# adrianstanea/UnitSpeech

Hardware: AMD Instinct MI355X
Metric: mel-frames/sec @ 50 diffusion steps, 80x1024 (higher is better)
Workload: dtype f32; 1 GPU; B=1 utterance(s)/GPU, 80x1024 mel, 50 diffusion steps, text+spk CFG (3 score evals/step), full-size decoder (119.1M params, synthetic weights), built-in Philox noise; batch_per_gpu=1, frames=1024, diffusion_steps=50, parallelism=utterance-sharded x1

## Files before the change

unitspeech_amd/csrc/conv_igemm.hip:

```cpp
#include <type_traits>
#include "kernels.h"
#include "pack_f16.h"

namespace us {

typedef float f32x16 __attribute__((ext_vector_type(16)));
typedef float f32x4 __attribute__((ext_vector_type(4)));
typedef _Float16 half8 __attribute__((ext_vector_type(8)));

constexpr int TN = 128;

__device__ __forceinline__ void blds16(__amdgpu_buffer_rsrc_t rsrc, unsigned voff_bytes, unsigned soff_bytes, float* lds_dst_wave_uniform) {
  __builtin_amdgcn_raw_ptr_buffer_load_lds(rsrc, (__attribute__((address_space(3))) void*)lds_dst_wave_uniform, 16, (int)voff_bytes,
                                           (int)soff_bytes, 0, 0);
}

template <int BK, int WM, bool WINO, bool F16 = false, int NWM = 2, int NSTG = 2, bool ASPLIT = false, int NB = 2>
__global__ __launch_bounds__(NWM * 128, 2) void conv_igemm_kernel(ConvArgs a) {
  constexpr int TN = 64 * NB;
  constexpr int NW = 2 * NWM;
  constexpr int TM = NWM * WM;
  constexpr int MB = WM / 32;
  constexpr int CPR = BK / 4;
  constexpr int RPI = 64 / CPR;
  constexpr int IA = TM / RPI / NW;
  constexpr int IB = TN / RPI / NW;
  static_assert(NSTG == 2 || NSTG == 3, "two or three operand buffers");
  constexpr int SWZ_DIV = 64 / BK;
  constexpr int BUF = (TM + TN) * BK;
  extern __shared__ __attribute__((aligned(16))) float smem[];

  const int tid = threadIdx.x, lane = tid & 63;
// ... 431 lines not shown
#pragma unroll
    for (int mb = 0; mb < MB; ++mb)
#pragma unroll
      for (int r = 0; r < 16; ++r) {
        const int m = m0 + wm * WM + mb * 32 + (r & 3) + 8 * (r >> 2) + 4 * hh;
        if (m < Ms) {
#pragma unroll
          for (int nb = 0; nb < NB; ++nb) {
            const int n = n0 + wn * (32 * NB) + nb * 32 + l32;
            if (n < a.Cout) slab[(long long)m * a.Cout + n] = acc[mb][nb][r];
          }
        }
      }
    return;
  }
  __syncthreads();
  if constexpr (!WINO && MB == 1 && NB == 2) {
    if (a.attn_part_ctx && n0 >= a.attn_q_cols) {
      const int h = ((n0 - a.attn_q_cols) / TN) * 2 + wn;
      float* xm = smem;
      float* xs = smem + 128;
      float* xc = smem + 256;
      const int mrow0 = m0 + wm * WM + 4 * hh;
      float kmax = -INFINITY;
#pragma unroll
      for (int mb = 0; mb < MB; ++mb)
#pragma unroll
        for (int r = 0; r < 16; ++r) {
          const bool ok = mrow0 + mb * 32 + (r & 3) + 8 * (r >> 2) < Ms;
          kmax = fmaxf(kmax, ok ? acc[mb][0][r] : -INFINITY);
// ... 28 lines not shown
        float* pc = a.attn_part_ctx + (blk * kHeads + h) * (kDimHead * kDimHead);
#pragma unroll
        for (int r = 0; r < 16; ++r) {
          const int d = (r & 3) + 8 * (r >> 2) + 4 * hh;
          pc[d * kDimHead + l32] = ctx[r] + xc[wn * 1024 + d * 32 + l32];
        }
        if (hh == 0) {
          a.attn_part_m[blk * kHidden + h * kDimHead + l32] = mcol;
          a.attn_part_s[blk * kHidden + h * kDimHead + l32] = ssum + xs[wn * 32 + l32];
        }
      }
      return;
    }
  }
  float* tr = smem + wave * (32 * 36);
  const bool need_xy = !dense || om_b != nullptr;
  const int trow = lane >> 3, tc4 = (lane & 7) * 4;
  const bool edge = WINO && (((a.Hout | a.Wout) & 1) != 0);
  bool out_over = false;
  float bias_col[NB];
  f32x4 bias_quad[NB];
#pragma unroll
  for (int nb = 0; nb < NB; ++nb) {
    const int ncol = n0 + wn * (32 * NB) + nb * 32;
    bias_col[nb] = (a.bias && ncol + l32 < a.Cout) ? a.bias[ncol + l32] : 0.f;
    bias_quad[nb] = f32x4{0.f, 0.f, 0.f, 0.f};
    if (a.bias && ncol + tc4 < a.Cout) bias_quad[nb] = *reinterpret_cast<const f32x4*>(a.bias + ncol + tc4);
  }
#pragma unroll
  for (int yi = 0; yi < NY; ++yi) {
  const f32x16 (&A)[MB][NB] = WINO ? Y[yi] : acc;
  const int oy0 = WINO ? (yi >> 1) : a_oy0, ox0 = WINO ? (yi & 1) : a_ox0;
#pragma unroll
  for (int mb = 0; mb < MB; ++mb) {
    const int m_base = m0 + wm * WM + mb * 32;
    int yb = 0, xb = 0;
    if (need_xy) { yb = m_base / a.Ws; xb = m_base - yb * a.Ws; }
#pragma unroll
    for (int nb = 0; nb < NB; ++nb) {
      const int ncol = n0 + wn * (32 * NB) + nb * 32;
      {
        const int n = ncol + l32;
// ... 17 lines not shown
#pragma unroll
      for (int k = 0; k < 4; ++k) {
        const int dr = trow + 8 * k;
        const int m = m_base + dr;
        f32x4 v = *reinterpret_cast<const f32x4*>(tr + dr * 36 + tc4);
        if (m < Ms && n < a.Cout) {
          int yy = yb, xx = xb + dr;
          if (need_xy) while (xx >= a.Ws) { xx -= a.Ws; ++yy; }
          const int ox = ox0 + xx * a.ostep;
          const int oy = oy0 + yy * a.ostep;
          if (edge && (oy >= a.Hout || ox >= a.Wout)) continue;
          const long long pix = dense ? (long long)m : (long long)oy * a.Wout + ox;
          v = v + b4;
          if (a.out2) *reinterpret_cast<f32x4*>(a.out2 + ((long long)b * a.Hout * a.Wout + pix) * a.out2_ld + n) = v;
          v = v * alpha;
          if (add_b) v += *reinterpret_cast<const f32x4*>(add_b + pix * a.add_ld + n);
          if (om_b) v *= om_b[ox * a.omask_step];
          if (a.out_split) {
            typedef _Float16 half4o __attribute__((ext_vector_type(4)));
            half4o hi, lo;
#pragma unroll
            for (int q = 0; q < 4; ++q) {
              us_half h_, l_;
              split_f16x3(v[q], h_, l_, out_over);
              hi[q] = h_;
              lo[q] = l_;
            }
            _Float16* oh = reinterpret_cast<_Float16*>(out_b + pix * a.out_ld) + 2 * (n & ~7) + (n & 7);
            *reinterpret_cast<half4o*>(oh) = hi;
            *reinterpret_cast<half4o*>(oh + 8) = lo;
          } else {
// ... 24 lines not shown
      }
    }
  }
#ifdef US_LIFE
  US_LIFE_AT(4);
  US_LIFE_AT(3);
  if (a.stamp_out && lane == 0) {
    unsigned long long* o = a.stamp_out + ((blockIdx.x + gridDim.x * blockIdx.z) * NW + wave) * 4;
    o[0] = life_t[0]; o[1] = life_t[1]; o[2] = life_t[2]; o[3] = life_t[3];
  }
#endif
}

__global__ __launch_bounds__(256) void splitk_finish_kernel(ConvArgs a) {
  __shared__ double s_g[kGroups][2];
  const int b = blockIdx.y;
  const int Ms = a.Hs * a.Ws;
  const int C4 = a.Cout >> 2;
  const long long total = (long long)Ms * C4;
  if (threadIdx.x < kGroups * 2) s_g[threadIdx.x >> 1][threadIdx.x & 1] = 0.0;
  __syncthreads();
  float t1[4] = {0.f, 0.f, 0.f, 0.f}, t2[4] = {0.f, 0.f, 0.f, 0.f};
  int tn = -1;
  const bool dense = (a.ostep == 1 && a.oy0 == 0 && a.ox0 == 0 && a.Hs == a.Hout && a.Ws == a.Wout);
  const float alpha = a.alpha ? *a.alpha : 1.f;
  float* out_b = a.out + (long long)b * a.Hout * a.Wout * a.out_ld;
  const float* add_b = a.add ? a.add + (long long)b * a.Hout * a.Wout * a.add_ld : nullptr;
  const float* om_b = a.omask ? a.omask + (long long)(b % a.omask_bmod) * a.omask_ld : nullptr;
  const long long slice = (long long)a.B * Ms * a.Cout;
  const int cg = a.Cout / kGroups;
  for (long long i = blockIdx.x * 256LL + threadIdx.x; i < total; i += (long long)gridDim.x * 256) {
    const int n = (int)(i % C4) * 4;
    const int m = (int)(i / C4);
    const float* p = a.splitk_ws + ((long long)b * Ms + m) * a.Cout + n;
    f32x4 v = *reinterpret_cast<const f32x4*>(p);
    int k = 1;
    for (; k + 8 <= a.ksplit; k += 8) {
      f32x4 u[8];
#pragma unroll
      for (int j = 0; j < 8; ++j) u[j] = *reinterpret_cast<const f32x4*>(p + (k + j) * slice);
#pragma unroll
      for (int j = 0; j < 8; ++j) v += u[j];
    }
// ... 5 lines not shown
        for (int k = 0; k < 4; ++k) {
          atomicAdd(&s_g[(tn + k) / cg][0], (double)t1[k]);
          atomicAdd(&s_g[(tn + k) / cg][1], (double)t2[k]);
          t1[k] = t2[k] = 0.f;
        }
      }
      tn = n;
#pragma unroll
      for (int k = 0; k < 4; ++k) { t1[k] += v[k]; t2[k] += v[k] * v[k]; }
    }
    const int yy = m / a.Ws, xx = m - yy * a.Ws;
    const int ox = a.ox0 + xx * a.ostep;
    const long long pix = dense ? (long long)m : (long long)(a.oy0 + yy * a.ostep) * a.Wout + ox;
    if (a.out2) *reinterpret_cast<f32x4*>(a.out2 + ((long long)b * a.Hout * a.Wout + pix) * a.out2_ld + n) = v;
    v *= alpha;
    if (add_b) v += *reinterpret_cast<const f32x4*>(add_b + pix * a.add_ld + n);
    if (om_b) v *= om_b[ox * a.omask_step];
    *reinterpret_cast<f32x4*>(out_b + pix * a.out_ld + n) = v;
  }
  if (a.stats) {
    if (tn >= 0) {
#pragma unroll
      for (int k = 0; k < 4; ++k) {
        atomicAdd(&s_g[(tn + k) / cg][0], (double)t1[k]);
        atomicAdd(&s_g[(tn + k) / cg][1], (double)t2[k]);
      }
    }
    __syncthreads();
    if (threadIdx.x < kGroups * 2)
      stat_add(a.stats, b, threadIdx.x >> 1, threadIdx.x & 1, blockIdx.x, s_g[threadIdx.x >> 1][threadIdx.x & 1]);
  }
// ... 10 lines not shown
hipError_t conv_igemm_init() {
  hipError_t e;
  if ((e = set_attr<32, 64, false>()) != hipSuccess) return e;
  if ((e = set_attr<32, 32, false>()) != hipSuccess) return e;
  if ((e = set_attr<16, 64, false>()) != hipSuccess) return e;
  if ((e = set_attr<16, 32, false>()) != hipSuccess) return e;
  if ((e = set_attr<32, 32, true>()) != hipSuccess) return e;
  if ((e = set_attr<32, 64, false, true>()) != hipSuccess) return e;
  if ((e = set_attr<32, 64, false, true, 4, 3>()) != hipSuccess) return e;
  if ((e = hipFuncSetAttribute(reinterpret_cast<const void*>(&conv_igemm_kernel<32, 64, false, true, 4, 3, false, 1>),
                               hipFuncAttributeMaxDynamicSharedMemorySize, (int)lds_bytes(32, 256, 3, 64))) != hipSuccess) return e;
  if ((e = set_attr<32, 64, false, true, 4, 3, true>()) != hipSuccess) return e;
  if ((e = set_attr<32, 64, false, true, 2, 2, true>()) != hipSuccess) return e;
  if ((e = set_attr<32, 32, false, true, 2, 2, true>()) != hipSuccess) return e;
  if ((e = set_attr<32, 32, false, true>()) != hipSuccess) return e;
  if ((e = set_attr<32, 32, true, true, 2, 3>()) != hipSuccess) return e;
  return set_attr<16, 32, true>();
}

hipError_t launch_conv_igemm(const ConvArgs& a_in, hipStream_t s) {
  ConvArgs a = a_in;
  a.range_flag = current_range_flag();
  if (a.B <= 0 || a.Hs <= 0 || a.Ws <= 0) return hipSuccess;
  if (!a.in || !a.wt || !a.out) return hipErrorInvalidValue;
  if ((a.bk != 16 && a.bk != 32) || a.Cin % a.bk != 0 || a.ntaps < 1 || a.ntaps > kMaxTaps) return hipErrorInvalidValue;
  if (a.in_ld % 4 != 0) return hipErrorInvalidValue;
  if (a.Cout % 4 != 0 || a.out_ld % 4 != 0 || (a.add && a.add_ld % 4 != 0)) return hipErrorInvalidValue;
  if ((long long)a.Hin * a.Win * a.in_ld * 4 >= (1LL << 31) || (long long)kMaxTaps * a.Cout * a.Cin * 4 >= (1LL << 31))
    return hipErrorInvalidValue;
  if (a.stats) {
    int cg = a.Cout / kGroups;
    if (a.Cout % kGroups != 0 || (cg & (cg - 1)) != 0) return hipErrorInvalidValue;
  }
  if (a.out2 && (a.out2_ld % 4 != 0 || a.wino_out || a.out_split || a.attn_part_ctx)) return hipErrorInvalidValue;
  const int Ms = a.Hs * a.Ws;
  int tn = TN;
  int nt = (a.Cout + TN - 1) / TN;
  int tm = a.tm;
  if (a.f16) {
    if (a.bk != 32) return hipErrorInvalidValue;
    if (a.f16 == 1 && !a.direct_presplit && a.ntaps == 1 && a.istride == 1 && !a.bias && !a.add) a.splitk_ws = nullptr;
    if (tm == 0) {
      if (a.f16 == 1 && (a.ntaps > 1 || a.direct_presplit)) {
        tm = (a.ntaps == 1 && a.nphase <= 1) || (long long)a.Hs * a.Ws < 512 ? 64 : 128;
      } else if (a.f16 == 1) {
        const long long per256 = (long long)((a.Hs * a.Ws + 255) / 256) * nt * a.B;
        const long long per128 = (long long)((a.Hs * a.Ws + 127) / 128) * nt * a.B;
        const long long cost256 = ((per256 + 255) / 256) * 256, cost128 = ((per128 + 255) / 256) * 128;
        constexpr int kTmModelMargin = 15;
// ... 35 lines not shown
  const int mt = (Ms + tm - 1) / tm;
  const long long tiles = (long long)mt * nt * a.B;
  const int S_all = a.ntaps * (a.Cin / a.bk);
  a.ksplit = 1;
  const long long tiles_item = a.splitk_by_batch ? tiles : (long long)mt * nt;
  if (a.splitk_ws && tiles_item < 128 && S_all >= 8 && a.Cout % 4 == 0 && a.out_ld % 4 == 0 && (!a.add || a.add_ld % 4 == 0)) {
    long long k = (256 + tiles_item - 1) / tiles_item;
    if (k > S_all / 4) k = S_all / 4;
    if (k > 512 / tiles_item) k = 512 / tiles_item;
    if (k > 32) k = 32;
    if (k >= 2 && k * (long long)a.B * Ms * a.Cout <= a.splitk_ws_floats) a.ksplit = (int)k;
  }
  a.nt = nt;
  dim3 grid(mt * a.ksplit * nt, 1, a.B * (a.nphase > 1 ? a.nphase : 1));
  const size_t lds = lds_bytes(a.bk, tm);
  if (a.f16 == 2) {
    if (tm == 256) hipLaunchKernelGGL((conv_igemm_kernel<32, 64, false, true, 4, 3, true>), grid, dim3(512), lds_bytes(32, 256, 3), s, a);
    else if (tm == 128) hipLaunchKernelGGL((conv_igemm_kernel<32, 64, false, true, 2, 2, true>), grid, dim3(256), lds, s, a);
    else hipLaunchKernelGGL((conv_igemm_kernel<32, 32, false, true, 2, 2, true>), grid, dim3(256), lds, s, a);
  } else if (a.f16) {
    if (a.wino_out) hipLaunchKernelGGL((conv_igemm_kernel<32, 32, true, true, 2, 3>), grid, dim3(256), lds_bytes(32, 64, 3), s, a);
    else if (tm == 256 && tn == 64) hipLaunchKernelGGL((conv_igemm_kernel<32, 64, false, true, 4, 3, false, 1>), grid, dim3(512), lds_bytes(32, 256, 3, 64), s, a);
    else if (tm == 256) hipLaunchKernelGGL((conv_igemm_kernel<32, 64, false, true, 4, 3>), grid, dim3(512), lds_bytes(32, 256, 3), s, a);
    else if (tm == 128) hipLaunchKernelGGL((conv_igemm_kernel<32, 64, false, true>), grid, dim3(256), lds, s, a);
    else hipLaunchKernelGGL((conv_igemm_kernel<32, 32, false, true>), grid, dim3(256), lds, s, a);
  } else if (a.wino_out) {
    if (a.bk == 32)
      hipLaunchKernelGGL((conv_igemm_kernel<32, 32, true>), grid, dim3(256), lds, s, a);
    else
      hipLaunchKernelGGL((conv_igemm_kernel<16, 32, true>), grid, dim3(256), lds, s, a);
  } else if (a.bk == 32 && tm == 128)
// ... 66 lines not shown
```

unitspeech_amd/csrc/decoder.hip:

```cpp
#include <hip/hip_runtime.h>

#include <cmath>
#include <cstdarg>
#include <cstdio>
#include <cstring>
#include <algorithm>
#include <map>
#include <memory>
#include <string>
#include <vector>

#include "../../include/unitspeech_hip.h"
#include "kernels.h"
#include "pack_f16.h"

using namespace us;

namespace {

thread_local std::string g_last_error;

struct DevBuf {
  float* p = nullptr;
  size_t n = 0;
// ... 73 lines not shown
  std::vector<int> C;
  struct Down { ResnetW r1, r2; AttnW a; bool has_ds; ResampleW ds; };
  struct Up { ResnetW r1, r2; AttnW a; ResampleW us; };
  std::vector<Down> downs;
  ResnetW mid1, mid2;
  AttnW mid_attn;
  std::vector<Up> ups;
  ConvW final_conv3;
  Slot *final_g, *final_b, *final_w1, *final_b1;
  Slot *text_uncon, *spk_uncon, *mlp0_w, *mlp0_b, *mlp2_w, *mlp2_b;
  int n_resnets = 0;
  int wino_min_level = 1;
  int wino4_level_form[8] = {0, 0, 0, 0, 0, 0, 0, 0};
  int wino_fuse = -1;
  bool wino_fuse_gn = true;
  int f16_tm = 0;
  int wgrad_side_streams = 1;
  std::vector<hipStream_t> wgrad_streams;
  std::vector<hipEvent_t> wgrad_events;
  bool training = false;
  float* zeros = nullptr;
  unsigned* range_flag = nullptr;
  unsigned* range_host = nullptr;
  bool exact = false;
  float* grad_scale = nullptr;
  CopyEnt* grad_tab_dev = nullptr;
  static constexpr size_t kLinJobs = 64;
  LinJob *lin_tab_dev = nullptr, *lin_tab_bwd_dev = nullptr;
  std::vector<CopyEnt> pending_copies;
  std::vector<PackJob> pending_packs;
// ... 442 lines not shown
  if (w.w->wino.p && e.b->wino_v) return in_split ? hipErrorInvalidValue : conv3x3_wino(e, w, in, in_ld, level, out, out_ld, stats);
  const int H = e.h->cfg.n_feats >> level, W = e.T >> level;
  ConvArgs a = base_args(e, w, in, in_ld, H, W, out, out_ld, H, W);
  if (in_split) {
    if (a.f16 != 2) return hipErrorInvalidValue;
    a.f16 = 1;
    a.direct_presplit = 1;
  }
  a.ntaps = 9;
  for (int ky = 0; ky < 3; ++ky)
    for (int kx = 0; kx < 3; ++kx) a.set_tap(ky * 3 + kx, ky - 1, kx - 1, ky * 3 + kx);
  a.stats = stats;
  return run_conv(e, a);
}

hipError_t conv1x1(EvalCtx& e, const ConvW& w, const float* in, int in_ld, int level, bool mask_out, float* out, int out_ld,
                   const float* add, int add_ld, const float* alpha, const float* wt_override, long long wt_bstride,
                   const float* bias_override, bool in_split = false, bool out_split = false, float* out2 = nullptr, int out2_ld = 0) {
  const int H = e.h->cfg.n_feats >> level, W = e.T >> level;
  ConvArgs a = base_args(e, w, in, in_ld, H, W, out, out_ld, H, W);
  a.out2 = out2; a.out2_ld = out2_ld;
  if (in_split) {
    if (a.f16 != 2) return hipErrorInvalidValue;
    a.f16 = 1;
    a.direct_presplit = 1;
  }
  a.out_split = out_split ? 1 : 0;
  a.ntaps = 1;
  a.set_tap(0, 0, 0, 0);
  if (mask_out) set_omask(e, a, level);
  a.add = add; a.add_ld = add_ld; a.alpha = alpha;
  if (wt_override) { a.wt = wt_override; a.wt_bstride = wt_bstride; a.bias = bias_override; }
  return run_conv(e, a);
}

hipError_t conv_down(EvalCtx& e, const ConvW& w, const float* in, int in_ld, int level, float* out, int out_ld, bool in_split = false) {
  const int H = e.h->cfg.n_feats >> level, W = e.T >> level;
  ConvArgs a = base_args(e, w, in, in_ld, H, W, out, out_ld, H / 2, W / 2);
  if (in_split) {
    if (a.f16 != 2) return hipErrorInvalidValue;
    a.f16 = 1;
    a.direct_presplit = 1;
  }
  a.ntaps = 9;
  a.istride = 2;
  for (int ky = 0; ky < 3; ++ky)
// ... 78 lines not shown
    WinoGnArgs g{};
    g.stats = st1; g.gamma = r.g1->buf.p; g.beta = r.b1->buf.p; g.temb = tproj;
    g.mask = e.mask; g.mask_ld = e.T; g.mask_step = 1 << l; g.mask_bmod = e.Bm;
    CK(conv3x3_wino(e, r.c2, S1, r.cout, l, S2, r.cout, st2, &g));
  } else {
    if (direct_presplit(e, r.c2, r.cout, out_ld) && out != in) {
      CK(gn_apply(e, S1, l, r.cout, st1, r.g1, r.b1, tproj, nullptr, 0, false, true, out, r.cout, true));
      CK(conv3x3(e, r.c2, out, r.cout, l, S2, r.cout, st2, true));
    } else {
      CK(gn_apply(e, S1, l, r.cout, st1, r.g1, r.b1, tproj, nullptr, 0, false, true, S1, r.cout));
      CK(conv3x3(e, r.c2, S1, r.cout, l, S2, r.cout, st2));
    }
  }
  if (R) {
    CK(gn_apply(e, S2, l, r.cout, st2, r.g2, r.b2, nullptr, R, r.cout, false, mask_out, out, out_ld, false, split_out));
  } else if (r.has_res) {
    CK(gn_apply(e, S2, l, r.cout, st2, r.g2, r.b2, nullptr, nullptr, 0, false, false, out, out_ld));
    CK(conv1x1(e, r.res, in, in_ld, l, mask_out, out, out_ld, out, out_ld, nullptr, nullptr, 0, nullptr, in_split));
  } else {
    CK(gn_apply(e, S2, l, r.cout, st2, r.g2, r.b2, nullptr, in, in_ld, false, mask_out, out, out_ld, false, split_out));
  }
  return hipSuccess;
}

inline bool next_takes_split_copy(EvalCtx& e, const ResnetW& r2) {
  return !e.h->exact && !r2.has_res && !r2.first && direct_presplit(e, r2.c1, r2.c1.cin, r2.c1.cin) &&
         r2.c1.cin == r2.cout;
}

inline bool resnet_takes_split(EvalCtx& e, const ResnetW& r) {
// ... 149 lines not shown
      else if (l <= L - 2) hid_split[l] = resnet_takes_split(e, h->ups[L - 1 - l].r1) && h->ups[L - 1 - l - 1].us.conv.w->direct_f16 ? 1 : 0;
    }
    for (int u = 0; u < L - 1; ++u) up_split[h->ups[u].r1.level] = h->ups[u].us.conv.w->direct_f16 ? 1 : 0;
    fin_split = L > 1 && !(h->final_conv3.w->wino.p && b.wino_v) && h->final_conv3.w->direct_f16 && h->ups[L - 2].us.conv.w->direct_f16;
  }
  const float* cur = nullptr;
  int cur_ld = 0;
  for (int l = 0; l < L; ++l) {
    auto& d = h->downs[l];
    const int c = h->C[l];
    const bool r2_copy = next_takes_split_copy(e, d.r2);
    if (l == 0) {
      const ResnetW& r = d.r1;
      double* st1 = next_stats(e);
      double* st2 = next_stats(e);
      CK(launch_first_conv(b.in2, r.c1.w->buf.p, r.c1.b->buf.p, r.res.w->buf.p, r.res.b->buf.p, b.S1[0], nullptr, st1, e.Bp, F, T, c, e.s));
      if (r.c2.w->wino.p && b.wino_v && h->wino_fuse_gn && gn_wino_input_supported(c)) {
        WinoGnArgs g{};
        g.stats = st1; g.gamma = r.g1->buf.p; g.beta = r.b1->buf.p; g.temb = b.tproj + b.tproj_off[r.index];
        g.mask = e.mask; g.mask_ld = e.T; g.mask_step = 1; g.mask_bmod = e.Bm;
        CK(conv3x3_wino(e, r.c2, b.S1[0], c, 0, b.S2[0], c, st2, &g));
      } else {
        if (direct_presplit(e, r.c2, c, c)) {
          CK(gn_apply(e, b.S1[0], 0, c, st1, r.g1, r.b1, b.tproj + b.tproj_off[r.index], nullptr, 0, false, true, b.P[0], c, true));
          CK(conv3x3(e, r.c2, b.P[0], c, 0, b.S2[0], c, st2, true));
        } else {
          CK(gn_apply(e, b.S1[0], 0, c, st1, r.g1, r.b1, b.tproj + b.tproj_off[r.index], nullptr, 0, false, true, b.S1[0], c));
          CK(conv3x3(e, r.c2, b.S1[0], c, 0, b.S2[0], c, st2));
        }
      }
      {
        GnApplyArgs ga;
// ... 192 lines not shown
    int cg = c / kGroups;
    if (cfg->dim_mults[i] < 1 || c % 16 != 0 || (cg & (cg - 1)) != 0) {
      g_last_error = "unsupported dim_mults (channels/8 must be a power of two)";
      return US_EINVAL;
    }
  }
  std::unique_ptr<us_decoder> h(new us_decoder());
  h->cfg = *cfg;
  if (hipGetDevice(&h->device) != hipSuccess) { g_last_error = "no HIP device"; return US_EHIP; }
  hipError_t e = conv_igemm_init();
  if (e != hipSuccess) { g_last_error = std::string("conv_igemm_init: ") + hipGetErrorString(e); return US_EHIP; }
  h->exact = (flags & US_CREATE_EXACT_FP32) != 0;
  if (const char* wl = getenv("US_WINO_MIN_LEVEL")) h->wino_min_level = atoi(wl);
  if (const char* wf = getenv("US_WINO_FUSE")) h->wino_fuse = atoi(wf) != 0 ? 1 : 0;
  if (const char* wf = getenv("US_WINO_FUSE_GN")) h->wino_fuse_gn = atoi(wf) != 0;
  if (const char* wt = getenv("US_F16_TM")) h->f16_tm = atoi(wt) == 64 || atoi(wt) == 128 || atoi(wt) == 256 ? atoi(wt) : 0;
  if (const char* ws = getenv("US_WGRAD_STREAM")) h->wgrad_side_streams = atoi(ws) < 0 ? 0 : (atoi(ws) > Tape::kSideMax ? Tape::kSideMax : atoi(ws));
  {
    const char* w4 = getenv("US_WINO4");
    std::string spec = w4 ? w4 : kWino4Default;
    size_t pos = 0;
    for (int l = 0; l < 8 && pos <= spec.size(); ++l) {
      const size_t comma = spec.find(',', pos);
      const std::string tok = spec.substr(pos, comma == std::string::npos ? std::string::npos : comma - pos);
      const int f = tok.empty() ? 0 : atoi(tok.c_str());
      h->wino4_level_form[l] = wino4_form_ok(f) ? f : 0;
      if (comma == std::string::npos) break;
      pos = comma + 1;
    }
    if (h->exact)
// ... 563 lines not shown
```

unitspeech_amd/csrc/kernels.h:

```cpp
#pragma once
#include <hip/hip_runtime.h>
#include <stdint.h>

namespace us {

#if defined(__HIPCC__)
__device__ __forceinline__ float mul_rn(float a, float b) {
#pragma clang fp contract(off)
  return a * b;
}
__device__ __forceinline__ float add_rn(float a, float b) {
#pragma clang fp contract(off)
  return a + b;
}
__device__ __forceinline__ float sub_rn(float a, float b) {
#pragma clang fp contract(off)
  return a - b;
}
#endif

constexpr float kF16Over = 65520.f;
enum : unsigned {
  kRangeAct = 1u,
  kRangeWeight = 2u,
// ... 54 lines not shown
  int nt;
  int f16;
  int wino_out;
  int splitk_by_batch;
  float* splitk_ws;
  long long splitk_ws_floats;
  unsigned* range_flag;
  int direct_presplit;
  int out_split;
  float* attn_part_ctx;
  float* attn_part_m;
  float* attn_part_s;
  int attn_nchunks;
  int attn_q_cols;
  int wt_rows;
  float* out2;
  int out2_ld;
#if defined(US_STAMP) || defined(US_LIFE)
  unsigned long long* stamp_out;
#endif
  unsigned long long dy_bits, dx_bits, wtap_bits;
  void set_tap(int i, int dy, int dx, int wtap) {
    dy_bits |= (unsigned long long)(dy + 8) << (4 * i);
    dx_bits |= (unsigned long long)(dx + 8) << (4 * i);
    wtap_bits |= (unsigned long long)wtap << (4 * i);
  }
  int nphase;
  unsigned long long ph_dy[4], ph_dx[4], ph_wtap[4];
  void set_phase_tap(int ph, int i, int dy, int dx, int wtap) {
    ph_dy[ph] |= (unsigned long long)(dy + 8) << (4 * i);
    ph_dx[ph] |= (unsigned long long)(dx + 8) << (4 * i);
    ph_wtap[ph] |= (unsigned long long)wtap << (4 * i);
  }
};
#if defined(__HIPCC__)
__device__ __forceinline__ void stat_add(double* stats, long long b, int group, int which, unsigned slot, double v) {
  atomicAdd(stats + ((b * kGroups + group) * 2 + which) * kStatSlots + (slot & (kStatSlots - 1)), v);
}
__device__ __forceinline__ double stat_read(const double* stats, long long b, int group, int which) {
  const double* p = stats + ((b * kGroups + group) * 2 + which) * kStatSlots;
  double t = 0.0;
#pragma unroll
  for (int i = 0; i < kStatSlots; ++i) t += p[i];
  return t;
}
#endif
inline int qkv_src_row(int cp) {
  if (cp < kHidden) return cp;
  const int t = cp - kHidden, h = t >> 6, w = t & 63;
  return (w < kDimHead ? kHidden : 2 * kHidden) + h * kDimHead + (w & (kDimHead - 1));
}
hipError_t launch_conv_igemm(const ConvArgs& a, hipStream_t s);
hipError_t conv_igemm_init();

hipError_t launch_pack_conv_weight(const float* src, float* dst, int Cout, int Cin, int KH, int KW, bool oihw, int bk,
                                   hipStream_t s, bool qkv_rows = false);
hipError_t launch_pack_conv_weight_f16(const float* src, float* dst, int Cout, int Cin, int KH, int KW, bool oihw, hipStream_t s,
                                       bool qkv_rows = false);

hipError_t launch_first_conv(const float* in2, const float* w3, const float* b3, const float* w1, const float* b1, float* y,
// ... 6 lines not shown
  const float* y; int y_ld;
  const double* stats;
  const float* gamma; const float* beta;
  const float* mask; int mask_ld, mask_step, mask_bmod;
  const float* temb; int temb_ld;
  const float* res; int res_ld; int res_masked;
  const float* res2_in; const float* res2_w; const float* res2_b;
  int post_mask;
  unsigned* range_flag;
  int out_split;
  float* out; int out_ld;
  float* out2; int out2_ld;
  int B, H, W, C;
};
hipError_t launch_gn_apply(const GnApplyArgs& a, hipStream_t s);
hipError_t launch_final_conv(const float* h, int ld, const float* w, const float* b0, const float* mask, int mask_ld,
                             int mask_bmod, float* out, int B, int H, int W, int C, hipStream_t s, const double* stats = nullptr,
                             const float* gamma = nullptr, const float* beta = nullptr);

hipError_t launch_attn_ctx_partial(const float* qkv, int B, int n, float* part_ctx, float* part_m, float* part_s, int nchunks,
                                   hipStream_t s);
constexpr int kAttnMaxSplit = 16;
hipError_t launch_attn_ctx_finalize(const float* part_ctx, const float* part_m, const float* part_s, int B, int nchunks,
                                    float* ctx, float* colM, float* colS, float* split_ws, hipStream_t s);
hipError_t launch_attn_wtotal(const float* ctx, const float* wout, const float* wq, float* wtotal, int B, int C, int bk, bool f16, hipStream_t s);
hipError_t launch_attn_weff(const float* ctx, const float* wout , float* weff, int B, int C, int bk, hipStream_t s,
                            bool f16 = false);
inline size_t attn_merge_scratch_floats(int B) { return (size_t)kAttnMaxSplit * B * kHeads * (kDimHead * kDimHead + 2 * kDimHead); }
hipError_t launch_attn_merge(const float* part_ctx, const float* part_m, const float* part_s, int B, int nchunks, float* ctx, float* colM,
                             float* colS, float* scratch, const float* wout, float* weff, int C, int bk, bool f16, hipStream_t s);
// ... 137 lines not shown
```

unitspeech_amd/csrc/ops.hip:

```cpp
#include "kernels.h"

namespace us {

typedef float f32x4 __attribute__((ext_vector_type(4)));

static thread_local unsigned* t_range_flag = nullptr;
unsigned* current_range_flag() { return t_range_flag; }
void set_range_flag(unsigned* p) { t_range_flag = p; }

__device__ __forceinline__ float wave_sum(float v) {
#pragma unroll
  for (int off = 32; off > 0; off >>= 1) v += __shfl_xor(v, off);
  return v;
}
__device__ __forceinline__ double wave_sum_d(double v) {
#pragma unroll
  for (int off = 32; off > 0; off >>= 1) v += __shfl_xor(v, off);
  return v;
}

__device__ __forceinline__ float mish_f(float x) {
  if (x > 20.f) return x;
  float w = __expf(x);
  float u = w * (w + 2.f);
  return x * (u * __builtin_amdgcn_rcpf(u + 2.f));
}

__global__ void stack_inputs_kernel(const float* __restrict__ x, int Bx, const float* __restrict__ mu, int Bmu, int n_text_uncond,
                                    const float* __restrict__ mu_feat, const float* __restrict__ mask, int Bm, float* __restrict__ in2,
                                    int Bp, int F, int T) {
  const long long total = (long long)Bp * F * T;
  for (long long i = blockIdx.x * (long long)blockDim.x + threadIdx.x; i < total; i += (long long)gridDim.x * blockDim.x) {
    int t = (int)(i % T);
    long long r = i / T;
    int f = (int)(r % F);
    int b = (int)(r / F);
    float m = mask[(long long)(b % Bm) * T + t];
    float xv = x[((long long)(b % Bx) * F + f) * T + t];
    float mv = b < n_text_uncond ? mu_feat[f] : mu[((long long)(b % Bmu) * F + f) * T + t];
    float2 o;
// ... 1 lines not shown
    o.y = xv * m;
    reinterpret_cast<float2*>(in2)[i] = o;
  }
}

hipError_t launch_stack_inputs(const float* x, int Bx, const float* mu, int Bmu, int n_text_uncond, const float* mu_feat,
                               const float* mask, int Bm, float* in2, int Bp, int F, int T, hipStream_t s) {
  long long total = (long long)Bp * F * T;
  int blocks = (int)((total + 255) / 256);
  if (blocks > 2048) blocks = 2048;
  hipLaunchKernelGGL(stack_inputs_kernel, dim3(blocks), dim3(256), 0, s, x, Bx, mu, Bmu, n_text_uncond, mu_feat, mask, Bm, in2, Bp, F, T);
  return hipGetLastError();
}

constexpr int FC_TW = 128;
__global__ __launch_bounds__(256) void first_conv_kernel(const float* __restrict__ in2, const float* __restrict__ w3,
                                                         const float* __restrict__ b3, const float* __restrict__ w1,
                                                         const float* __restrict__ b1, float* __restrict__ y, float* __restrict__ r,
                                                         double* __restrict__ stats, int F, int T, int C) {
  __shared__ __attribute__((aligned(8))) float patch[3][FC_TW + 2][2];
  __shared__ double gred[kGroups][2];
  if (threadIdx.x < kGroups * 2) gred[threadIdx.x >> 1][threadIdx.x & 1] = 0.0;
  const int b = blockIdx.z, f = blockIdx.y, t0 = blockIdx.x * FC_TW;
  const int tid = threadIdx.x;
  for (int i = tid; i < 3 * (FC_TW + 2) * 2; i += 256) {
    int c = i & 1, xx = (i >> 1) % (FC_TW + 2), yy = (i >> 1) / (FC_TW + 2);
    int ff = f + yy - 1, tt = t0 + xx - 1;
    float v = 0.f;
    if (ff >= 0 && ff < F && tt >= 0 && tt < T) v = in2[(((long long)b * F + ff) * T + tt) * 2 + c];
    patch[yy][xx][c] = v;
  }
  __syncthreads();
  const int C4 = C >> 2;
  const int qpb = C4 < 256 ? C4 : 256;
  const int nrun = 256 / qpb;
  const int flen = (FC_TW + nrun - 1) / nrun;
  const int run = tid / qpb, ql = tid - run * qpb;
  const int cg = C / kGroups;
  typedef float f32x2 __attribute__((ext_vector_type(2)));
  if (run < nrun) {
    for (int q = ql; q < C4; q += qpb) {
      const int co = 4 * q;
      float w[4][18];
      f32x4 bb, r0, r1, rb;
#pragma unroll
      for (int k = 0; k < 4; ++k) {
#pragma unroll
        for (int i = 0; i < 18; ++i) w[k][i] = w3[(co + k) * 18 + i];
        bb[k] = b3[co + k]; r0[k] = w1[(co + k) * 2]; r1[k] = w1[(co + k) * 2 + 1]; rb[k] = b1[co + k];
      }
      f32x4 s1 = {0.f, 0.f, 0.f, 0.f}, s2 = s1;
      const int xlo = run * flen, xhi = (xlo + flen < FC_TW ? xlo + flen : FC_TW);
      f32x2 win[3][3];
#pragma unroll
      for (int ky = 0; ky < 3; ++ky) {
        win[ky][1] = *reinterpret_cast<const f32x2*>(&patch[ky][xlo][0]);
        win[ky][2] = *reinterpret_cast<const f32x2*>(&patch[ky][xlo + 1][0]);
      }
      for (int xx = xlo; xx < xhi; ++xx) {
        if (t0 + xx >= T) break;
#pragma unroll
        for (int ky = 0; ky < 3; ++ky) {
          win[ky][0] = win[ky][1];
          win[ky][1] = win[ky][2];
          win[ky][2] = *reinterpret_cast<const f32x2*>(&patch[ky][xx + 2][0]);
        }
        f32x4 acc = bb;
#pragma unroll
        for (int ci = 0; ci < 2; ++ci)
#pragma unroll
          for (int ky = 0; ky < 3; ++ky)
#pragma unroll
            for (int kx = 0; kx < 3; ++kx)
#pragma unroll
              for (int k = 0; k < 4; ++k) acc[k] = fmaf(w[k][ci * 9 + ky * 3 + kx], win[ky][kx][ci], acc[k]);
        const long long p = ((long long)b * F + f) * T + t0 + xx;
        *reinterpret_cast<f32x4*>(y + p * C + co) = acc;
        s1 += acc;
        s2 += acc * acc;
        if (r) {
          f32x4 rv;
#pragma unroll
          for (int k = 0; k < 4; ++k) rv[k] = fmaf(r1[k], win[1][1][1], fmaf(r0[k], win[1][1][0], rb[k]));
          *reinterpret_cast<f32x4*>(r + p * C + co) = rv;
        }
      }
      if (stats) {
#pragma unroll
        for (int k = 0; k < 4; ++k) {
          atomicAdd(&gred[(co + k) / cg][0], (double)s1[k]);
          atomicAdd(&gred[(co + k) / cg][1], (double)s2[k]);
        }
      }
    }
  }
  if (stats) {
    __syncthreads();
    if (threadIdx.x < kGroups * 2)
      stat_add(stats, b, threadIdx.x >> 1, threadIdx.x & 1, blockIdx.x + blockIdx.y * gridDim.x, gred[threadIdx.x >> 1][threadIdx.x & 1]);
  }
}

hipError_t launch_first_conv(const float* in2, const float* w3, const float* b3, const float* w1, const float* b1, float* y,
                             float* r, double* stats, int Bp, int F, int T, int C, hipStream_t s) {
  if (C % 4 != 0) return hipErrorInvalidValue;
  dim3 grid((T + FC_TW - 1) / FC_TW, F, Bp);
  hipLaunchKernelGGL(first_conv_kernel, grid, dim3(256), 0, s, in2, w3, b3, w1, b1, y, r, stats, F, T, C);
  return hipGetLastError();
}

__global__ __launch_bounds__(256) void gn_stats_kernel(const float* __restrict__ y, int ld, int n, int C, double* __restrict__ stats) {
  __shared__ double red[kGroups][2];
  const int b = blockIdx.y, tid = threadIdx.x;
  if (tid < kGroups * 2) red[tid >> 1][tid & 1] = 0.0;
  __syncthreads();
  const int cg = C / kGroups;
  const long long total = (long long)n * C;
  const float* yb = y + (long long)b * n * ld;
  double s1[kGroups], s2[kGroups];
#pragma unroll
  for (int g = 0; g < kGroups; ++g) s1[g] = s2[g] = 0.0;
  for (long long i = blockIdx.x * 256LL + tid; i < total; i += (long long)gridDim.x * 256) {
// ... 18 lines not shown
  long long total = (long long)n * C;
  int blocks = (int)((total + 256 * 16 - 1) / (256 * 16));
  if (blocks < 1) blocks = 1;
  if (blocks > 512) blocks = 512;
  hipLaunchKernelGGL(gn_stats_kernel, dim3(blocks, B), dim3(256), 0, s, y, ld, n, C, stats);
  return hipGetLastError();
}

__global__ __launch_bounds__(256) void gn_apply_kernel(GnApplyArgs a) {
  const int b = blockIdx.y;
  const int C4 = a.C >> 2;
  const int cg = a.C / kGroups;
  const long long n = (long long)a.H * a.W;
  const double cnt = (double)n * cg;
  __shared__ float s_mean[kGroups], s_rstd[kGroups];
  if (threadIdx.x < kGroups) {
    double mean = stat_read(a.stats, b, threadIdx.x, 0) / cnt;
    double var = stat_read(a.stats, b, threadIdx.x, 1) / cnt - mean * mean;
    if (var < 0) var = 0;
    s_mean[threadIdx.x] = (float)mean;
    s_rstd[threadIdx.x] = (float)(1.0 / sqrt(var + 1e-5));
  }
  __syncthreads();
  const float* yb = a.y + (long long)b * n * a.y_ld;
  float* ob = a.out + (long long)b * n * a.out_ld;
  float* o2b = a.out2 ? a.out2 + (long long)b * n * a.out2_ld : nullptr;
  const float* rb = a.res ? a.res + (long long)b * n * a.res_ld : nullptr;
  const float* mb = a.mask + (long long)(b % a.mask_bmod) * a.mask_ld;
  const float* tb = a.temb ? a.temb + (long long)b * a.temb_ld : nullptr;
  const long long total = n * C4;
  const long long stride = (long long)gridDim.x * 256;
  long long i = blockIdx.x * 256LL + threadIdx.x;
  const bool fixed_quad = (stride % C4) == 0;
  bool over = false;
  int c = (int)(i % C4) * 4;
  f32x4 sc, sh, te = {0.f, 0.f, 0.f, 0.f};
  f32x4 r2w0 = {0.f, 0.f, 0.f, 0.f}, r2w1 = r2w0, r2b = r2w0;
// ... 458 lines not shown
```

Measured before the change: 3197 mel-frames/s.

## Fuse GroupNorm+Mish apply into residual 1x1 conv epilogue and recompute first conv

In inference, the second GroupNorm+Mish of resnet blocks with a residual 1x1 conv is now applied inside that conv's epilogue (and its split-K finish), removing a separate gn_apply pass and its intermediate write and read. The first decoder conv gains a stats-only mode that skips storing its output, then a second pass recomputes the cheap 3x3 conv and applies GN, Mish, temb and mask directly, optionally writing split-f16 output for the next conv. This trades extra recomputation and a heavier conv epilogue (per-pixel index math, mish) for fewer memory passes and launches. Both paths are controlled by an env flag that is on by default.

```diff
diff --git a/unitspeech_amd/csrc/conv_igemm.hip b/unitspeech_amd/csrc/conv_igemm.hip
--- a/unitspeech_amd/csrc/conv_igemm.hip
+++ b/unitspeech_amd/csrc/conv_igemm.hip
@@ -15,7 +15,7 @@
                                            (int)soff_bytes, 0, 0);
 }
 
-template <int BK, int WM, bool WINO, bool F16 = false, int NWM = 2, int NSTG = 2, bool ASPLIT = false, int NB = 2>
+template <int BK, int WM, bool WINO, bool F16 = false, int NWM = 2, int NSTG = 2, bool ASPLIT = false, int NB = 2, bool GNADD = false>
 __global__ __launch_bounds__(NWM * 128, 2) void conv_igemm_kernel(ConvArgs a) {
   constexpr int TN = 64 * NB;
   constexpr int NW = 2 * NWM;
@@ -477,6 +477,13 @@
       }
     return;
   }
+  float (*gn_ms)[2] = nullptr;
+  if constexpr (GNADD) {
+    __shared__ float gn_ms_lds[kGroups][2];
+    gn_ms = gn_ms_lds;
+    if (threadIdx.x < kGroups)
+      gn_group_stats(a.gn_stats, b, threadIdx.x, (double)a.Hout * a.Wout * (a.Cout / kGroups), gn_ms[threadIdx.x][0], gn_ms[threadIdx.x][1]);
+  }
   __syncthreads();
   if constexpr (!WINO && MB == 1 && NB == 2) {
     if (a.attn_part_ctx && n0 >= a.attn_q_cols) {
@@ -535,7 +542,7 @@
     }
   }
   float* tr = smem + wave * (32 * 36);
-  const bool need_xy = !dense || om_b != nullptr;
+  const bool need_xy = !dense || om_b != nullptr || GNADD;
   const int trow = lane >> 3, tc4 = (lane & 7) * 4;
   const bool edge = WINO && (((a.Hout | a.Wout) & 1) != 0);
   bool out_over = false;
@@ -547,6 +554,29 @@
     bias_col[nb] = (a.bias && ncol + l32 < a.Cout) ? a.bias[ncol + l32] : 0.f;
     bias_quad[nb] = f32x4{0.f, 0.f, 0.f, 0.f};
     if (a.bias && ncol + tc4 < a.Cout) bias_quad[nb] = *reinterpret_cast<const f32x4*>(a.bias + ncol + tc4);
+  }
+  f32x4 gn_sc[NB], gn_sh[NB];
+  const float* gny_b = nullptr;
+  const float* gnm_b = nullptr;
+  if constexpr (GNADD) {
+    gny_b = a.gn_y + (long long)b * a.Hout * a.Wout * a.gn_y_ld;
+    gnm_b = a.gn_mask + (long long)(b % a.omask_bmod) * a.omask_ld;
+    const int cg = a.Cout / kGroups;
+#pragma unroll
+    for (int nb = 0; nb < NB; ++nb) {
+      const int n = n0 + wn * (32 * NB) + nb * 32 + tc4;
+      gn_sc[nb] = gn_sh[nb] = f32x4{0.f, 0.f, 0.f, 0.f};
+      if (n < a.Cout) {
+        const f32x4 ga = *reinterpret_cast<const f32x4*>(a.gn_gamma + n);
+        const f32x4 be = *reinterpret_cast<const f32x4*>(a.gn_beta + n);
+#pragma unroll
+        for (int k = 0; k < 4; ++k) {
+          const int gk = (n + k) / cg;
+          gn_sc[nb][k] = gn_ms[gk][1] * ga[k];
+          gn_sh[nb][k] = be[k] - gn_ms[gk][0] * gn_sc[nb][k];
+        }
+      }
+    }
   }
 #pragma unroll
   for (int yi = 0; yi < NY; ++yi) {
@@ -594,7 +624,16 @@
           v = v + b4;
           if (a.out2) *reinterpret_cast<f32x4*>(a.out2 + ((long long)b * a.Hout * a.Wout + pix) * a.out2_ld + n) = v;
           v = v * alpha;
-          if (add_b) v += *reinterpret_cast<const f32x4*>(add_b + pix * a.add_ld + n);
+          if constexpr (GNADD) {
+            const f32x4 y4 = *reinterpret_cast<const f32x4*>(gny_b + pix * a.gn_y_ld + n);
+            const float gm = gnm_b[ox * a.omask_step];
+            f32x4 h4;
+#pragma unroll
+            for (int q = 0; q < 4; ++q) h4[q] = mish_f(y4[q] * gn_sc[nb][q] + gn_sh[nb][q]) * gm;
+            v += h4;
+          } else {
+            if (add_b) v += *reinterpret_cast<const f32x4*>(add_b + pix * a.add_ld + n);
+          }
           if (om_b) v *= om_b[ox * a.omask_step];
           if (a.out_split) {
             typedef _Float16 half4o __attribute__((ext_vector_type(4)));
@@ -649,11 +688,14 @@
 
 __global__ __launch_bounds__(256) void splitk_finish_kernel(ConvArgs a) {
   __shared__ double s_g[kGroups][2];
+  __shared__ float gn_ms[kGroups][2];
   const int b = blockIdx.y;
   const int Ms = a.Hs * a.Ws;
   const int C4 = a.Cout >> 2;
   const long long total = (long long)Ms * C4;
   if (threadIdx.x < kGroups * 2) s_g[threadIdx.x >> 1][threadIdx.x & 1] = 0.0;
+  if (a.gn_y && threadIdx.x < kGroups)
+    gn_group_stats(a.gn_stats, b, threadIdx.x, (double)a.Hout * a.Wout * (a.Cout / kGroups), gn_ms[threadIdx.x][0], gn_ms[threadIdx.x][1]);
   __syncthreads();
   float t1[4] = {0.f, 0.f, 0.f, 0.f}, t2[4] = {0.f, 0.f, 0.f, 0.f};
   int tn = -1;
@@ -662,6 +704,8 @@
   float* out_b = a.out + (long long)b * a.Hout * a.Wout * a.out_ld;
   const float* add_b = a.add ? a.add + (long long)b * a.Hout * a.Wout * a.add_ld : nullptr;
   const float* om_b = a.omask ? a.omask + (long long)(b % a.omask_bmod) * a.omask_ld : nullptr;
+  const float* gny_b = a.gn_y ? a.gn_y + (long long)b * a.Hout * a.Wout * a.gn_y_ld : nullptr;
+  const float* gnm_b = a.gn_y ? a.gn_mask + (long long)(b % a.omask_bmod) * a.omask_ld : nullptr;
   const long long slice = (long long)a.B * Ms * a.Cout;
   const int cg = a.Cout / kGroups;
   for (long long i = blockIdx.x * 256LL + threadIdx.x; i < total; i += (long long)gridDim.x * 256) {
@@ -697,7 +741,23 @@
     const long long pix = dense ? (long long)m : (long long)(a.oy0 + yy * a.ostep) * a.Wout + ox;
     if (a.out2) *reinterpret_cast<f32x4*>(a.out2 + ((long long)b * a.Hout * a.Wout + pix) * a.out2_ld + n) = v;
     v *= alpha;
-    if (add_b) v += *reinterpret_cast<const f32x4*>(add_b + pix * a.add_ld + n);
+    if (gny_b) {
+      const f32x4 y4 = *reinterpret_cast<const f32x4*>(gny_b + pix * a.gn_y_ld + n);
+      const f32x4 ga = *reinterpret_cast<const f32x4*>(a.gn_gamma + n);
+      const f32x4 be = *reinterpret_cast<const f32x4*>(a.gn_beta + n);
+      const float gm = gnm_b[ox * a.omask_step];
+      f32x4 h4;
+#pragma unroll
+      for (int q = 0; q < 4; ++q) {
+        const int gk = (n + q) / cg;
+        const float sc = gn_ms[gk][1] * ga[q];
+        const float sh = be[q] - gn_ms[gk][0] * sc;
+        h4[q] = mish_f(y4[q] * sc + sh) * gm;
+      }
+      v += h4;
+    } else if (add_b) {
+      v += *reinterpret_cast<const f32x4*>(add_b + pix * a.add_ld + n);
+    }
     if (om_b) v *= om_b[ox * a.omask_step];
     *reinterpret_cast<f32x4*>(out_b + pix * a.out_ld + n) = v;
   }
@@ -738,6 +798,10 @@
   if ((e = set_attr<32, 64, false, true, 2, 2, true>()) != hipSuccess) return e;
   if ((e = set_attr<32, 32, false, true, 2, 2, true>()) != hipSuccess) return e;
   if ((e = set_attr<32, 32, false, true>()) != hipSuccess) return e;
+  if ((e = hipFuncSetAttribute(reinterpret_cast<const void*>(&conv_igemm_kernel<32, 32, false, true, 2, 2, true, 2, true>),
+                               hipFuncAttributeMaxDynamicSharedMemorySize, (int)lds_bytes(32, 64))) != hipSuccess) return e;
+  if ((e = hipFuncSetAttribute(reinterpret_cast<const void*>(&conv_igemm_kernel<32, 32, false, true, 2, 2, false, 2, true>),
+                               hipFuncAttributeMaxDynamicSharedMemorySize, (int)lds_bytes(32, 64))) != hipSuccess) return e;
   if ((e = set_attr<32, 32, true, true, 2, 3>()) != hipSuccess) return e;
   return set_attr<16, 32, true>();
 }
@@ -757,6 +821,12 @@
     if (a.Cout % kGroups != 0 || (cg & (cg - 1)) != 0) return hipErrorInvalidValue;
   }
   if (a.out2 && (a.out2_ld % 4 != 0 || a.wino_out || a.out_split || a.attn_part_ctx)) return hipErrorInvalidValue;
+  if (a.gn_y) {
+    if (!a.gn_stats || !a.gn_gamma || !a.gn_beta || !a.gn_mask || a.gn_y_ld % 4 != 0 || a.add || a.wino_out || a.attn_part_ctx ||
+        a.nphase > 1 || !a.f16 || a.tm != 0 || a.ntaps != 1 || a.istride != 1 || a.ostep != 1 || a.oy0 != 0 || a.ox0 != 0 ||
+        a.Hs != a.Hout || a.Ws != a.Wout || a.Cout % kGroups != 0 || a.omask_bmod < 1 || (a.f16 == 1 && !a.direct_presplit))
+      return hipErrorInvalidValue;
+  }
   const int Ms = a.Hs * a.Ws;
   int tn = TN;
   int nt = (a.Cout + TN - 1) / TN;
@@ -822,7 +892,12 @@
   a.nt = nt;
   dim3 grid(mt * a.ksplit * nt, 1, a.B * (a.nphase > 1 ? a.nphase : 1));
   const size_t lds = lds_bytes(a.bk, tm);
-  if (a.f16 == 2) {
+  if (a.gn_y && tm != 64) return hipErrorInvalidValue;
+  if (a.gn_y && a.f16 == 2) {
+    hipLaunchKernelGGL((conv_igemm_kernel<32, 32, false, true, 2, 2, true, 2, true>), grid, dim3(256), lds, s, a);
+  } else if (a.gn_y) {
+    hipLaunchKernelGGL((conv_igemm_kernel<32, 32, false, true, 2, 2, false, 2, true>), grid, dim3(256), lds, s, a);
+  } else if (a.f16 == 2) {
     if (tm == 256) hipLaunchKernelGGL((conv_igemm_kernel<32, 64, false, true, 4, 3, true>), grid, dim3(512), lds_bytes(32, 256, 3), s, a);
     else if (tm == 128) hipLaunchKernelGGL((conv_igemm_kernel<32, 64, false, true, 2, 2, true>), grid, dim3(256), lds, s, a);
     else hipLaunchKernelGGL((conv_igemm_kernel<32, 32, false, true, 2, 2, true>), grid, dim3(256), lds, s, a);
diff --git a/unitspeech_amd/csrc/decoder.hip b/unitspeech_amd/csrc/decoder.hip
--- a/unitspeech_amd/csrc/decoder.hip
+++ b/unitspeech_amd/csrc/decoder.hip
@@ -111,6 +111,7 @@
   int wino4_level_form[8] = {0, 0, 0, 0, 0, 0, 0, 0};
   int wino_fuse = -1;
   bool wino_fuse_gn = true;
+  bool gn_pass_fusion = true;
   int f16_tm = 0;
   int wgrad_side_streams = 1;
   std::vector<hipStream_t> wgrad_streams;
@@ -583,9 +584,16 @@
   return run_conv(e, a);
 }
 
+struct ConvGnAdd {
+  const float* y; int y_ld;
+  const double* stats;
+  const Slot* gamma; const Slot* beta;
+};
+
 hipError_t conv1x1(EvalCtx& e, const ConvW& w, const float* in, int in_ld, int level, bool mask_out, float* out, int out_ld,
                    const float* add, int add_ld, const float* alpha, const float* wt_override, long long wt_bstride,
-                   const float* bias_override, bool in_split = false, bool out_split = false, float* out2 = nullptr, int out2_ld = 0) {
+                   const float* bias_override, bool in_split = false, bool out_split = false, float* out2 = nullptr, int out2_ld = 0,
+                   const ConvGnAdd* gn_add = nullptr) {
   const int H = e.h->cfg.n_feats >> level, W = e.T >> level;
   ConvArgs a = base_args(e, w, in, in_ld, H, W, out, out_ld, H, W);
   a.out2 = out2; a.out2_ld = out2_ld;
@@ -599,6 +607,11 @@
   a.set_tap(0, 0, 0, 0);
   if (mask_out) set_omask(e, a, level);
   a.add = add; a.add_ld = add_ld; a.alpha = alpha;
+  if (gn_add) {
+    a.gn_y = gn_add->y; a.gn_y_ld = gn_add->y_ld; a.gn_stats = gn_add->stats;
+    a.gn_gamma = gn_add->gamma->buf.p; a.gn_beta = gn_add->beta->buf.p;
+    a.gn_mask = e.mask; a.omask_ld = e.T; a.omask_step = 1 << level; a.omask_bmod = e.Bm;
+  }
   if (wt_override) { a.wt = wt_override; a.wt_bstride = wt_bstride; a.bias = bias_override; }
   return run_conv(e, a);
 }
@@ -707,6 +720,9 @@
   }
   if (R) {
     CK(gn_apply(e, S2, l, r.cout, st2, r.g2, r.b2, nullptr, R, r.cout, false, mask_out, out, out_ld, false, split_out));
+  } else if (r.has_res && e.infer && e.h->gn_pass_fusion && r.res.w->direct_f16) {
+    const ConvGnAdd ga{S2, r.cout, st2, r.g2, r.b2};
+    CK(conv1x1(e, r.res, in, in_ld, l, mask_out, out, out_ld, nullptr, 0, nullptr, nullptr, 0, nullptr, in_split, false, nullptr, 0, &ga));
   } else if (r.has_res) {
     CK(gn_apply(e, S2, l, r.cout, st2, r.g2, r.b2, nullptr, nullptr, 0, false, false, out, out_ld));
     CK(conv1x1(e, r.res, in, in_ld, l, mask_out, out, out_ld, out, out_ld, nullptr, nullptr, 0, nullptr, in_split));
@@ -886,8 +902,24 @@
       const ResnetW& r = d.r1;
       double* st1 = next_stats(e);
       double* st2 = next_stats(e);
-      CK(launch_first_conv(b.in2, r.c1.w->buf.p, r.c1.b->buf.p, r.res.w->buf.p, r.res.b->buf.p, b.S1[0], nullptr, st1, e.Bp, F, T, c, e.s));
-      if (r.c2.w->wino.p && b.wino_v && h->wino_fuse_gn && gn_wino_input_supported(c)) {
+      const bool wino_gn = r.c2.w->wino.p && b.wino_v && h->wino_fuse_gn && gn_wino_input_supported(c);
+      const bool recompute = e.infer && h->gn_pass_fusion && !wino_gn;
+      CK(launch_first_conv(b.in2, r.c1.w->buf.p, r.c1.b->buf.p, r.res.w->buf.p, r.res.b->buf.p, recompute ? nullptr : b.S1[0], nullptr, st1,
+                           e.Bp, F, T, c, e.s));
+      if (recompute) {
+        const bool split = direct_presplit(e, r.c2, c, c);
+        GnApplyArgs ga;
+        memset(&ga, 0, sizeof ga);
+        ga.stats = st1; ga.gamma = r.g1->buf.p; ga.beta = r.b1->buf.p;
+        ga.mask = e.mask; ga.mask_ld = e.T; ga.mask_step = 1; ga.mask_bmod = e.Bm;
+        ga.temb = b.tproj + b.tproj_off[r.index]; ga.temb_ld = c;
+        ga.post_mask = 1;
+        ga.out_split = split ? 1 : 0;
+        ga.out = split ? b.P[0] : b.S1[0]; ga.out_ld = c;
+        ga.B = e.Bp; ga.H = F; ga.W = T; ga.C = c;
+        CK(launch_first_conv_gn(b.in2, r.c1.w->buf.p, r.c1.b->buf.p, ga, e.s));
+        CK(conv3x3(e, r.c2, ga.out, c, 0, b.S2[0], c, st2, split));
+      } else if (wino_gn) {
         WinoGnArgs g{};
         g.stats = st1; g.gamma = r.g1->buf.p; g.beta = r.b1->buf.p; g.temb = b.tproj + b.tproj_off[r.index];
         g.mask = e.mask; g.mask_ld = e.T; g.mask_step = 1; g.mask_bmod = e.Bm;
@@ -1110,6 +1142,7 @@
   if (const char* wl = getenv("US_WINO_MIN_LEVEL")) h->wino_min_level = atoi(wl);
   if (const char* wf = getenv("US_WINO_FUSE")) h->wino_fuse = atoi(wf) != 0 ? 1 : 0;
   if (const char* wf = getenv("US_WINO_FUSE_GN")) h->wino_fuse_gn = atoi(wf) != 0;
+  if (const char* gf = getenv("US_GN_PASS_FUSION")) h->gn_pass_fusion = atoi(gf) != 0;
   if (const char* wt = getenv("US_F16_TM")) h->f16_tm = atoi(wt) == 64 || atoi(wt) == 128 || atoi(wt) == 256 ? atoi(wt) : 0;
   if (const char* ws = getenv("US_WGRAD_STREAM")) h->wgrad_side_streams = atoi(ws) < 0 ? 0 : (atoi(ws) > Tape::kSideMax ? Tape::kSideMax : atoi(ws));
   {
diff --git a/unitspeech_amd/csrc/kernels.h b/unitspeech_amd/csrc/kernels.h
--- a/unitspeech_amd/csrc/kernels.h
+++ b/unitspeech_amd/csrc/kernels.h
@@ -92,6 +92,10 @@
   int attn_nchunks;
   int attn_q_cols;
   int wt_rows;
+  const float* gn_y; int gn_y_ld;
+  const double* gn_stats;
+  const float* gn_gamma; const float* gn_beta;
+  const float* gn_mask;
   float* out2;
   int out2_ld;
 #if defined(US_STAMP) || defined(US_LIFE)
@@ -122,6 +126,19 @@
   for (int i = 0; i < kStatSlots; ++i) t += p[i];
   return t;
 }
+__device__ __forceinline__ void gn_group_stats(const double* stats, long long b, int group, double cnt, float& mean_out, float& rstd_out) {
+  double mean = stat_read(stats, b, group, 0) / cnt;
+  double var = stat_read(stats, b, group, 1) / cnt - mean * mean;
+  if (var < 0) var = 0;
+  mean_out = (float)mean;
+  rstd_out = (float)(1.0 / sqrt(var + 1e-5));
+}
+__device__ __forceinline__ float mish_f(float x) {
+  if (x > 20.f) return x;
+  float w = __expf(x);
+  float u = w * (w + 2.f);
+  return x * (u * __builtin_amdgcn_rcpf(u + 2.f));
+}
 #endif
 inline int qkv_src_row(int cp) {
   if (cp < kHidden) return cp;
@@ -158,6 +175,7 @@
   int B, H, W, C;
 };
 hipError_t launch_gn_apply(const GnApplyArgs& a, hipStream_t s);
+hipError_t launch_first_conv_gn(const float* in2, const float* w3, const float* b3, const GnApplyArgs& a, hipStream_t s);
 hipError_t launch_final_conv(const float* h, int ld, const float* w, const float* b0, const float* mask, int mask_ld,
                              int mask_bmod, float* out, int B, int H, int W, int C, hipStream_t s, const double* stats = nullptr,
                              const float* gamma = nullptr, const float* beta = nullptr);
diff --git a/unitspeech_amd/csrc/ops.hip b/unitspeech_amd/csrc/ops.hip
--- a/unitspeech_amd/csrc/ops.hip
+++ b/unitspeech_amd/csrc/ops.hip
@@ -17,13 +17,6 @@
 #pragma unroll
   for (int off = 32; off > 0; off >>= 1) v += __shfl_xor(v, off);
   return v;
-}
-
-__device__ __forceinline__ float mish_f(float x) {
-  if (x > 20.f) return x;
-  float w = __expf(x);
-  float u = w * (w + 2.f);
-  return x * (u * __builtin_amdgcn_rcpf(u + 2.f));
 }
 
 __global__ void stack_inputs_kernel(const float* __restrict__ x, int Bx, const float* __restrict__ mu, int Bmu, int n_text_uncond,
@@ -55,15 +48,29 @@
 }
 
 constexpr int FC_TW = 128;
+enum { kFcStore = 0, kFcStats = 1, kFcGn = 2 };
+struct FirstConvGn {
+  const double* stats;
+  const float* gamma; const float* beta;
+  const float* temb; int temb_ld;
+  const float* mask; int mask_ld, mask_bmod;
+  float* out; int out_ld; int out_split;
+  unsigned* range_flag;
+};
+template <int MODE>
 __global__ __launch_bounds__(256) void first_conv_kernel(const float* __restrict__ in2, const float* __restrict__ w3,
                                                          const float* __restrict__ b3, const float* __restrict__ w1,
                                                          const float* __restrict__ b1, float* __restrict__ y, float* __restrict__ r,
-                                                         double* __restrict__ stats, int F, int T, int C) {
+                                                         double* __restrict__ stats, int F, int T, int C, FirstConvGn g) {
   __shared__ __attribute__((aligned(8))) float patch[3][FC_TW + 2][2];
   __shared__ double gred[kGroups][2];
+  __shared__ float s_mean[kGroups], s_rstd[kGroups];
   if (threadIdx.x < kGroups * 2) gred[threadIdx.x >> 1][threadIdx.x & 1] = 0.0;
   const int b = blockIdx.z, f = blockIdx.y, t0 = blockIdx.x * FC_TW;
   const int tid = threadIdx.x;
+  if constexpr (MODE == kFcGn) {
+    if (tid < kGroups) gn_group_stats(g.stats, b, tid, (double)F * T * (C / kGroups), s_mean[tid], s_rstd[tid]);
+  }
   for (int i = tid; i < 3 * (FC_TW + 2) * 2; i += 256) {
     int c = i & 1, xx = (i >> 1) % (FC_TW + 2), yy = (i >> 1) / (FC_TW + 2);
     int ff = f + yy - 1, tt = t0 + xx - 1;
@@ -72,6 +79,7 @@
     patch[yy][xx][c] = v;
   }
   __syncthreads();
+  bool over = false;
   const int C4 = C >> 2;
   const int qpb = C4 < 256 ? C4 : 256;
   const int nrun = 256 / qpb;
@@ -91,6 +99,18 @@
         bb[k] = b3[co + k]; r0[k] = w1[(co + k) * 2]; r1[k] = w1[(co + k) * 2 + 1]; rb[k] = b1[co + k];
       }
       f32x4 s1 = {0.f, 0.f, 0.f, 0.f}, s2 = s1;
+      f32x4 sc = s1, sh = s1, te = s1;
+      if constexpr (MODE == kFcGn) {
+        const f32x4 ga = *reinterpret_cast<const f32x4*>(g.gamma + co);
+        const f32x4 be = *reinterpret_cast<const f32x4*>(g.beta + co);
+#pragma unroll
+        for (int k = 0; k < 4; ++k) {
+          const int gk = (co + k) / cg;
+          sc[k] = s_rstd[gk] * ga[k];
+          sh[k] = be[k] - s_mean[gk] * sc[k];
+        }
+        if (g.temb) te = *reinterpret_cast<const f32x4*>(g.temb + (long long)b * g.temb_ld + co);
+      }
       const int xlo = run * flen, xhi = (xlo + flen < FC_TW ? xlo + flen : FC_TW);
       f32x2 win[3][3];
 #pragma unroll
@@ -116,17 +136,42 @@
 #pragma unroll
               for (int k = 0; k < 4; ++k) acc[k] = fmaf(w[k][ci * 9 + ky * 3 + kx], win[ky][kx][ci], acc[k]);
         const long long p = ((long long)b * F + f) * T + t0 + xx;
-        *reinterpret_cast<f32x4*>(y + p * C + co) = acc;
+        if constexpr (MODE == kFcGn) {
+          const float m = g.mask[(long long)(b % g.mask_bmod) * g.mask_ld + t0 + xx];
+          f32x4 o;
+#pragma unroll
+          for (int k = 0; k < 4; ++k) o[k] = mish_f(acc[k] * sc[k] + sh[k]) * m;
+          o += te;
+          o *= m;
+          if (g.out_split) {
+            typedef _Float16 half4_t __attribute__((ext_vector_type(4)));
+            half4_t hi, lo;
+#pragma unroll
+            for (int k = 0; k < 4; ++k) {
+              us_half h, l;
+              split_f16x3(o[k], h, l, over);
+              hi[k] = h;
+              lo[k] = l;
+            }
+            _Float16* oh = reinterpret_cast<_Float16*>(g.out + p * g.out_ld) + 2 * (co & ~7) + (co & 7);
+            *reinterpret_cast<half4_t*>(oh) = hi;
+            *reinterpret_cast<half4_t*>(oh + 8) = lo;
+          } else {
+            *reinterpret_cast<f32x4*>(g.out + p * g.out_ld + co) = o;
+          }
+          continue;
+        }
+        if constexpr (MODE == kFcStore) *reinterpret_cast<f32x4*>(y + p * C + co) = acc;
         s1 += acc;
         s2 += acc * acc;
-        if (r) {
+        if (MODE == kFcStore && r) {
           f32x4 rv;
 #pragma unroll
           for (int k = 0; k < 4; ++k) rv[k] = fmaf(r1[k], win[1][1][1], fmaf(r0[k], win[1][1][0], rb[k]));
           *reinterpret_cast<f32x4*>(r + p * C + co) = rv;
         }
       }
-      if (stats) {
+      if (MODE != kFcGn && stats) {
 #pragma unroll
         for (int k = 0; k < 4; ++k) {
           atomicAdd(&gred[(co + k) / cg][0], (double)s1[k]);
@@ -135,6 +180,10 @@
       }
     }
   }
+  if constexpr (MODE == kFcGn) {
+    if (g.out_split) range_report(g.range_flag, over, kRangeAct);
+    return;
+  }
   if (stats) {
     __syncthreads();
     if (threadIdx.x < kGroups * 2)
@@ -145,8 +194,28 @@
 hipError_t launch_first_conv(const float* in2, const float* w3, const float* b3, const float* w1, const float* b1, float* y,
                              float* r, double* stats, int Bp, int F, int T, int C, hipStream_t s) {
   if (C % 4 != 0) return hipErrorInvalidValue;
+  if (!y && (r || !stats)) return hipErrorInvalidValue;
   dim3 grid((T + FC_TW - 1) / FC_TW, F, Bp);
-  hipLaunchKernelGGL(first_conv_kernel, grid, dim3(256), 0, s, in2, w3, b3, w1, b1, y, r, stats, F, T, C);
+  FirstConvGn g{};
+  if (y) hipLaunchKernelGGL(first_conv_kernel<kFcStore>, grid, dim3(256), 0, s, in2, w3, b3, w1, b1, y, r, stats, F, T, C, g);
+  else hipLaunchKernelGGL(first_conv_kernel<kFcStats>, grid, dim3(256), 0, s, in2, w3, b3, w1, b1, y, r, stats, F, T, C, g);
+  return hipGetLastError();
+}
+
+hipError_t launch_first_conv_gn(const float* in2, const float* w3, const float* b3, const GnApplyArgs& a, hipStream_t s) {
+  if (a.C % 4 != 0 || a.C % kGroups != 0 || a.out_ld % 4 != 0 || !a.stats || !a.mask || !a.out || !a.post_mask || a.mask_step != 1 ||
+      a.res || a.res2_in || a.out2 || a.mask_bmod < 1)
+    return hipErrorInvalidValue;
+  if (a.out_split && (a.C % 8 != 0 || a.out_ld % 8 != 0)) return hipErrorInvalidValue;
+  FirstConvGn g{};
+  g.stats = a.stats; g.gamma = a.gamma; g.beta = a.beta;
+  g.temb = a.temb; g.temb_ld = a.temb_ld;
+  g.mask = a.mask; g.mask_ld = a.mask_ld; g.mask_bmod = a.mask_bmod;
+  g.out = a.out; g.out_ld = a.out_ld; g.out_split = a.out_split;
+  g.range_flag = current_range_flag();
+  dim3 grid((a.W + FC_TW - 1) / FC_TW, a.H, a.B);
+  hipLaunchKernelGGL(first_conv_kernel<kFcGn>, grid, dim3(256), 0, s, in2, w3, b3, nullptr, nullptr, nullptr, nullptr, nullptr, a.H, a.W,
+                     a.C, g);
   return hipGetLastError();
 }
 
@@ -195,13 +264,7 @@
   const long long n = (long long)a.H * a.W;
   const double cnt = (double)n * cg;
   __shared__ float s_mean[kGroups], s_rstd[kGroups];
-  if (threadIdx.x < kGroups) {
-    double mean = stat_read(a.stats, b, threadIdx.x, 0) / cnt;
-    double var = stat_read(a.stats, b, threadIdx.x, 1) / cnt - mean * mean;
-    if (var < 0) var = 0;
-    s_mean[threadIdx.x] = (float)mean;
-    s_rstd[threadIdx.x] = (float)(1.0 / sqrt(var + 1e-5));
-  }
+  if (threadIdx.x < kGroups) gn_group_stats(a.stats, b, threadIdx.x, cnt, s_mean[threadIdx.x], s_rstd[threadIdx.x]);
   __syncthreads();
   const float* yb = a.y + (long long)b * n * a.y_ld;
   float* ob = a.out + (long long)b * n * a.out_ld;
```

Result: no change. 3227 mel-frames/s, median of 6 (+0.9%).
